# yml-bit/CTA-GAN

Measured on AMD Instinct MI355X. Metric: paired 512x512 slices/sec (G+D step); generator rel-L2 vs CPU reference, higher is better.
Workload: dtype bf16; 1 GPU; HdGan stage-2 full G+D train step (G, Reg, STN, D_m, losses, Adam x3), 16 paired 512x512 slices/GPU; per_gpu_batch=16, global_batch=16, size=512, parallelism=single, rccl_ranks=1, dp_backend=none

## Files before the change

### cta_gan_amd/csrc/conv_halo.h

```cpp
#pragma once
#include <stdlib.h>
#include <type_traits>
#include "common.h"
#include "conv_dispatch.h"

struct ConvArgs {
    const void* x;
    const void* w;
    void* y;
    const float* bias;
    int B, Hi, Wi, Cin, x_ld;
    int Ho, Wo, Cout, y_ld;
    int Hs, Ws, oy0, ox0, os, is;
    int frame;
    int pad_mode, act;
    int w_tap_stride;
    int ntaps;
    int taps[64];
    int kh, kw, dy0, dx0;
    float* stats;
    const void* res;
    const void* fold;
    int res_ld, fold_ld;
    const void* bz;
// ... 490 lines not shown
                                add_bf16x8(f, q); add_bf16x8(f, q + f_lo);
                            }
                        }
                    }
                    bf16x8 hi, lo;
#pragma unroll
                    for (int e = 0; e < 8; ++e) {
                        hi[e] = (bf16_t)f[e];
                        lo[e] = (bf16_t)(f[e] - (float)hi[e]);
                    }
                    bf16_t* yp = Y + (((size_t)n * a.Ho + (oy * a.os + oy0_)) * a.Wo + (ox * a.os + ox0_)) * a.y_ld + n0 + chl;
                    *reinterpret_cast<bf16x8*>(yp) = hi;
                    *reinterpret_cast<bf16x8*>(yp + y_lo) = lo;
                    if constexpr (FUSE) {
                        if (bst) {
                            const bf16_t* zp = Z + (((size_t)n * a.Hs + oy) * a.Ws + ox) * a.bz_ld + n0 + chl;
                            float zf[8];
#pragma unroll
                            for (int e = 0; e < 8; ++e) zf[e] = 0.f;
                            add_bf16x8(zf, zp);
                            add_bf16x8(zf, zp + z_lo);
#pragma unroll
                            for (int e = 0; e < 8; ++e) {
                                const float xh = (zf[e] - bmu[e]) * brs[e];
                                float gg = (float)hi[e] + (float)lo[e];
                                if (a.bact == ACT_RELU) gg = xh > 0.f ? gg : 0.f;
                                else if (a.bact == ACT_LRELU) gg = xh > 0.f ? gg : LRELU_SLOPE * gg;
                                bs1[e] += gg;
                                bs2[e] += gg * xh;
                            }
                        }
                    }
                }
            }
            if constexpr (FUSE) {
                if (bst) {
                    __syncthreads();
                    float* red = reinterpret_cast<float*>(smem);
#pragma unroll
                    for (int e = 0; e < 8; ++e) { red[tid * 16 + e] = bs1[e]; red[tid * 16 + 8 + e] = bs2[e]; }
                    __syncthreads();
                    const int ntile = gridDim.x / ntn;
                    for (int cl = tid; cl < CR; cl += NTH) {
                        const int ch = chan_of(cl, rd);
                        if (n0 + ch < a.Cout) {
                            float t1 = 0.f, t2 = 0.f;
                            for (int q = 0; q < NTH / CPR; ++q) {
                                const float* r = red + (q * CPR + (cl >> 3)) * 16 + (cl & 7);
                                t1 += r[0];
                                t2 += r[8];
                            }
                            float* dst = a.bstats + (((size_t)n * ntile + spc) * a.Cout + n0 + ch) * 2;
                            dst[0] = t1;
                            dst[1] = t2;
                        }
                    }
                }
            }
        }
    } else if constexpr (sizeof(OutT) == 2) {
        constexpr int RS = BN * 2 + 16;
        char* st = smem;
#pragma unroll
        for (int nt = 0; nt < TN; ++nt) {
            const int co = (wn * TN + nt) * 16 + co_l;
            float bv[4];
#pragma unroll
            for (int r = 0; r < 4; ++r)
                bv[r] = (a.bias != nullptr && n0 + co + r < a.Cout) ? a.bias[n0 + co + r] : 0.f;
#pragma unroll
            for (int mt = 0; mt < TM; ++mt) {
                const int prow = (wm * TM + mt) * HALO_W + (lane & 15);
                bf16x4 o;
#pragma unroll
                for (int r = 0; r < 4; ++r) {
                    if constexpr (NIE) o[r] = (bf16_t)act_apply((acc[mt][nt][r] - nmr[nt][r]) * nrr[nt][r], a.nie_act);
                    else o[r] = (bf16_t)act_apply(acc[mt][nt][r] + bv[r], a.act);
                }
                *reinterpret_cast<bf16x4*>(st + prow * RS + co * 2) = o;
            }
        }
        OutT* __restrict__ Y = (OutT*)a.y;
        const bf16_t* __restrict__ R = (const bf16_t*)a.res;
        const bf16_t* __restrict__ F = (const bf16_t*)a.fold;
        constexpr int CPR = BN / 8;
        constexpr int NIT = BM * CPR / NTH;
        u32x4 rv[FUSE ? NIT : 1], zv[FUSE ? NIT : 1];
        if constexpr (FUSE) {
#pragma unroll
            for (int it = 0; it < NIT; ++it) {
                const int cidx = tid + NTH * it;
                const int prow = cidx / CPR, ch = (cidx % CPR) * 8;
                const int oy = y0 + prow / HALO_W, ox = x0 + prow % HALO_W;
                const bool ok = R != nullptr && oy < a.Hs && ox < a.Ws && n0 + ch < a.Cout;
                rv[it] = *reinterpret_cast<const u32x4*>(
                    ok ? R + (((size_t)n * a.Hs + oy) * a.Ws + ox) * a.res_ld + n0 + ch : (const bf16_t*)g_zero_chunk);
                const bool okz = a.bstats != nullptr && oy < a.Hs && ox < a.Ws && n0 + ch < a.Cout;
                zv[it] = *reinterpret_cast<const u32x4*>(
                    okz ? (const bf16_t*)a.bz + (((size_t)n * a.Hs + oy) * a.Ws + ox) * a.bz_ld + n0 + ch : (const bf16_t*)g_zero_chunk);
            }
        }
        const bool bst = FUSE && a.bstats != nullptr;
        float bs1[8], bs2[8], bmu[8], brs[8];
#pragma unroll
        for (int e = 0; e < 8; ++e) { bs1[e] = 0.f; bs2[e] = 0.f; bmu[e] = 0.f; brs[e] = 0.f; }
        if constexpr (FUSE) {
            static_assert(NTH % CPR == 0, "a thread keeps its channel chunk over the store loop");
            const int chl = (tid % CPR) * 8;
            if (bst && n0 + chl < a.Cout) {
#pragma unroll
                for (int e = 0; e < 8; ++e) {
                    bmu[e] = a.bmean[(size_t)n * a.Cout + n0 + chl + e];
                    brs[e] = a.brstd[(size_t)n * a.Cout + n0 + chl + e];
                }
            }
        }
        __syncthreads();
#pragma unroll
        for (int it = 0; it < NIT; ++it) {
            const int cidx = tid + NTH * it;
            const int prow = cidx / CPR, ch = (cidx % CPR) * 8;
            const int oy = y0 + prow / HALO_W, ox = x0 + prow % HALO_W;
            if (oy < a.Hs && ox < a.Ws && n0 + ch < a.Cout) {
                OutT* yp = Y + (((size_t)n * a.Ho + (oy * a.os + oy0_)) * a.Wo + (ox * a.os + ox0_)) * a.y_ld + n0 + ch;
                u32x4 v = *reinterpret_cast<const u32x4*>(st + prow * RS + ch * 2);
                if constexpr (FUSE) {
                    float f[8], g[8];
                    unpack_bf16x8(v, f);
                    unpack_bf16x8(rv[it], g);
#pragma unroll
                    for (int e = 0; e < 8; ++e) f[e] += g[e];
                    if (F != nullptr) {
                        const int ey = oy == 1 ? 0 : (oy == a.Hs - 2 ? a.Hs + 1 : -1);
                        const int ex = ox == 1 ? 0 : (ox == a.Ws - 2 ? a.Ws + 1 : -1);
                        const OutT* Fn = F + (size_t)n * (a.Hs + 2) * (a.Ws + 2) * a.fold_ld + n0 + ch;
                        if (ey >= 0) add_bf16x8(f, Fn + ((size_t)ey * (a.Ws + 2) + ox + 1) * a.fold_ld);
                        if (ex >= 0) add_bf16x8(f, Fn + ((size_t)(oy + 1) * (a.Ws + 2) + ex) * a.fold_ld);
                        if (ey >= 0 && ex >= 0) add_bf16x8(f, Fn + ((size_t)ey * (a.Ws + 2) + ex) * a.fold_ld);
                    }
                    bf16x8 o;
#pragma unroll
                    for (int e = 0; e < 8; ++e) o[e] = (bf16_t)f[e];
                    v = __builtin_bit_cast(u32x4, o);
                    if (bst) {
                        float zf[8];
                        unpack_bf16x8(zv[it], zf);
#pragma unroll
                        for (int e = 0; e < 8; ++e) {
                            const float xh = (zf[e] - bmu[e]) * brs[e];
                            float gg = (float)o[e];
                            if (a.bact == ACT_RELU) gg = xh > 0.f ? gg : 0.f;
                            else if (a.bact == ACT_LRELU) gg = xh > 0.f ? gg : LRELU_SLOPE * gg;
                            bs1[e] += gg;
                            bs2[e] += gg * xh;
                        }
                    }
                }
                *reinterpret_cast<u32x4*>(yp) = v;
            }
        }
        if constexpr (FUSE) {
            if (bst) {
                __syncthreads();
                float* red = reinterpret_cast<float*>(smem);
#pragma unroll
                for (int e = 0; e < 8; ++e) { red[tid * 16 + e] = bs1[e]; red[tid * 16 + 8 + e] = bs2[e]; }
                __syncthreads();
                const int ntile = gridDim.x / ntn;
                for (int cl = tid; cl < BN; cl += NTH) {
                    if (n0 + cl < a.Cout) {
                        float t1 = 0.f, t2 = 0.f;
                        for (int q = 0; q < NTH / CPR; ++q) {
                            const float* r = red + (q * CPR + (cl >> 3)) * 16 + (cl & 7);
                            t1 += r[0];
                            t2 += r[8];
                        }
                        float* dst = a.bstats + (((size_t)n * ntile + spc) * a.Cout + n0 + cl) * 2;
                        dst[0] = t1;
                        dst[1] = t2;
                    }
                }
            }
        }
    } else {
        OutT* __restrict__ Y = (OutT*)a.y;
        const bool vec_ok = ((a.Cout & 3) == 0) && ((a.y_ld & 3) == 0);
#pragma unroll
        for (int mt = 0; mt < TM; ++mt) {
            const int oy = y0 + wm * TM + mt, ox = x0 + (lane & 15);
            if (oy >= a.Hs || ox >= a.Ws) continue;
            OutT* yp = Y + (((size_t)n * a.Ho + (oy * a.os + oy0_)) * a.Wo + (ox * a.os + ox0_)) * a.y_ld;
#pragma unroll
            for (int nt = 0; nt < TN; ++nt) {
                const int co = n0 + (wn * TN + nt) * 16 + co_l;
                if (co >= a.Cout) continue;
                float v[4];
#pragma unroll
                for (int r = 0; r < 4; ++r) {
                    const float b = (a.bias != nullptr && co + r < a.Cout) ? a.bias[co + r] : 0.f;
                    v[r] = act_apply(acc[mt][nt][r] + b, a.act);
                }
                if (FUSE && a.res != nullptr) {
                    const float* rp = (const float*)a.res + (((size_t)n * a.Hs + oy) * a.Ws + ox) * a.res_ld + co;
#pragma unroll
                    for (int r = 0; r < 4; ++r)
                        if (co + r < a.Cout) v[r] += rp[r];
                }
                if (FUSE && a.fold != nullptr) {
                    const int ey = oy == 1 ? 0 : (oy == a.Hs - 2 ? a.Hs + 1 : -1);
                    const int ex = ox == 1 ? 0 : (ox == a.Ws - 2 ? a.Ws + 1 : -1);
                    const float* Fn = (const float*)a.fold + (size_t)n * (a.Hs + 2) * (a.Ws + 2) * a.fold_ld + co;
#pragma unroll
                    for (int r = 0; r < 4; ++r) {
                        if (co + r >= a.Cout) continue;
                        if (ey >= 0) v[r] += Fn[((size_t)ey * (a.Ws + 2) + ox + 1) * a.fold_ld + r];
                        if (ex >= 0) v[r] += Fn[((size_t)(oy + 1) * (a.Ws + 2) + ex) * a.fold_ld + r];
                        if (ey >= 0 && ex >= 0) v[r] += Fn[((size_t)ey * (a.Ws + 2) + ex) * a.fold_ld + r];
                    }
                }
                if (vec_ok) {
                    *reinterpret_cast<f32x4*>(yp + co) = f32x4{v[0], v[1], v[2], v[3]};
                } else {
#pragma unroll
                    for (int r = 0; r < 4; ++r)
                        if (co + r < a.Cout) yp[co + r] = v[r];
                }
            }
        }
    }
}

template <typename T, typename OutT, int BN, int WM, int WN, int KCH, int ABUF, int TH = 16, bool FUSE = false, int KWC = 0, bool MC = false, bool PK = false,
          bool S2D = false, bool NIE = false>
static int launch_halo_cfg(const ConvArgs& a, hipStream_t st, int* tiles_out = nullptr) {
    if constexpr (!NIE && KWC == 3 && (TH == 16 || (TH == 8 && !PK)) && BN == 128 && WM == 4 && WN == 2 && KCH == 8 && !MC && !S2D &&
                  sizeof(T) == 2 && ((std::is_same<OutT, bf16_t>::value && !PK) || (std::is_same<OutT, bfpair_t>::value && PK))) {
        if (a.nie_sync != nullptr) {
            if ((FUSE && (a.fold != nullptr || a.bstats != nullptr)) || a.stats == nullptr || a.Cout % BN) return CTG_EINVAL;
            return launch_halo_cfg<T, OutT, BN, WM, WN, KCH, ABUF, TH, FUSE, KWC, false, PK, false, true>(a, st, tiles_out);
        }
    }
    if constexpr (!S2D && !FUSE && !MC && KWC == 0 && TH == 16 && sizeof(T) == 2 && KCH == 8 && BN >= 64 && !std::is_same<OutT, float>::value) {
        if (a.s2d) {
            if (a.res != nullptr || a.fold != nullptr) return -1;
            return launch_halo_cfg<T, OutT, BN, WM, WN, KCH, ABUF, TH, false, 0, false, PK, true>(a, st, tiles_out);
        }
    }
    if (a.s2d && !S2D) return -1;
    if constexpr (!FUSE && !MC && !S2D && !NIE) {
        if (a.res != nullptr || a.fold != nullptr) return launch_halo_cfg<T, OutT, BN, WM, WN, KCH, ABUF, TH, true, KWC, false, PK>(a, st, tiles_out);
    }
    if constexpr (!MC && !S2D && !FUSE && KWC == 0 && (TH == 16 || (TH == 8 && BN == 64)) && sizeof(T) == 2 &&
                  ((std::is_same<OutT, bf16_t>::value && !PK) || (std::is_same<OutT, bfpair_t>::value && PK))) {
        if (a.ncls == 4) return launch_halo_cfg<T, OutT, BN, WM, WN, KCH, ABUF, TH, false, 0, true, PK>(a, st, tiles_out);
    }
    if constexpr (KWC == 0 && !MC && !S2D && sizeof(T) == 2) {
        if (a.kw == 3 && a.kh <= 3 && a.ncls <= 1) return launch_halo_cfg<T, OutT, BN, WM, WN, KCH, ABUF, TH, FUSE, 3, false, PK>(a, st, tiles_out);
    }
    if (a.ncls > 1 && !MC && !S2D) return -1;
    if (a.nie_sync != nullptr && !NIE) return CTG_EINVAL;
    constexpr int NTH = WM * WN * 64;
    const int hpw = HALO_W + a.kw - 1, hph = TH + a.kh - 1;
    const int hpc = hph * hpw * KCH;
    const int hpc64 = (hpc + 63) & ~63;
    const int epc = VecOf<T>::N;
    const int nchunk = a.Cin / (KCH * epc);
    const int main_lds = (((nchunk > 1 && ABUF == 2) ? 2 : 1) * hpc64 + 2 * BN * KCH) * 16;
    const int epi_lds = std::is_same<OutT, bfpair_t>::value ? TH * HALO_W * ((BN / WN) * 4 + 16)
                        : sizeof(OutT) == 2 ? TH * HALO_W * (BN * 2 + 16) : 0;
    if (FUSE && a.bstats != nullptr && WM * WN * 64 * 64 > (main_lds > epi_lds ? main_lds : epi_lds)) return -1;
    const int smem = main_lds > epi_lds ? main_lds : epi_lds;
    if (smem > 160 * 1024 || hph * hpw >= 65536) return -1;
    static unsigned long long attr_mask = 0;
    {
        const int rc = ctg_lds_attr_once((const void*)conv_halo_kernel<T, OutT, BN, WM, WN, KCH, ABUF, TH, FUSE, KWC, MC, PK, S2D, NIE>,
                                         160 * 1024, &attr_mask);
        if (rc != CTG_OK) return rc;
    }
    const int tiles = ((a.Hs + TH - 1) / TH) * ((a.Ws + HALO_W - 1) / HALO_W) * (MC ? 4 : 1);
    if (tiles_out != nullptr) *tiles_out = tiles;
    const int ntn = (a.Cout + BN - 1) / BN;
    if constexpr (NIE) {
        static int occ_dev[64];
        int dev = 0;
        if (hipGetDevice(&dev) != hipSuccess) dev = 0;
        dev &= 63;
        if (occ_dev[dev] == 0) {
            int occ = 0;
            if (hipOccupancyMaxActiveBlocksPerMultiprocessor(
                    &occ, (const void*)conv_halo_kernel<T, OutT, BN, WM, WN, KCH, ABUF, TH, FUSE, KWC, MC, PK, S2D, NIE>, NTH, smem) != hipSuccess ||
                occ < 1)
                occ = 1;
            occ_dev[dev] = occ;
        }
        const int share = ctg_knobs().nie_share > 0 ? ctg_knobs().nie_share : 2;
        if ((long)tiles * ntn * share > (long)occ_dev[dev] * ctg_cu_count()) return 2;
    }
    dim3 grid(tiles * ntn, a.B);
    hipLaunchKernelGGL((conv_halo_kernel<T, OutT, BN, WM, WN, KCH, ABUF, TH, FUSE, KWC, MC, PK, S2D, NIE>), grid, dim3(NTH), smem, st, a);
    return ctg_launch_status();
}

static int launch_strip32(const ConvArgs& a, hipStream_t st, int* tiles_out, bool pair);

template <typename T, int KCH>
static int launch_halo_t(const ConvArgs& a, int out_f32, hipStream_t st, int* tiles_out) {
    if (a.is != 1 && !a.s2d) return -1;
    if (out_f32 >= 2) {
        if constexpr (sizeof(T) == 2 && KCH == 8) {
            if (out_f32 == 2) {
                if (a.Cout > 64) return launch_halo_cfg<T, bfpair_t, 128, 4, 2, 8, 1, 16, false, 0, false, true>(a, st, tiles_out);
                if (a.Cout > 32) {
                    if (a.ncls == 4 && !ctg_knobs().no_mc_th8) return launch_halo_cfg<T, bfpair_t, 64, 4, 1, 8, 1, 8, false, 0, false, true>(a, st, tiles_out);
                    if (!ctg_knobs().no_th8_64 && a.ncls <= 1 && a.Hs >= 16)
                        return launch_halo_cfg<T, bfpair_t, 64, 4, 1, 8, 1, 8, false, 0, false, true>(a, st, tiles_out);
                    return launch_halo_cfg<T, bfpair_t, 64, 4, 1, 8, 1, 16, false, 0, false, true>(a, st, tiles_out);
                }
                if (a.Cout > 16) {
                    const int rc = launch_strip32(a, st, tiles_out, true);
                    if (rc != -1) return rc;
                    return launch_halo_cfg<T, bfpair_t, 32, 4, 1, 8, 1, 16, false, 0, false, true>(a, st, tiles_out);
                }
                return -1;
            }
            if (a.Cout > 64) return launch_halo_cfg<T, float, 128, 4, 2, 8, 1, 16, false, 0, false, true>(a, st, tiles_out);
            if (a.Cout > 32) return launch_halo_cfg<T, float, 64, 4, 1, 8, 1, 16, false, 0, false, true>(a, st, tiles_out);
            if (a.Cout > 16) return launch_halo_cfg<T, float, 32, 4, 1, 8, 1, 16, false, 0, false, true>(a, st, tiles_out);
            return launch_halo_cfg<T, float, 16, 4, 1, 8, 1, 16, false, 0, false, true>(a, st, tiles_out);
        }
        return -1;
    }
    if (a.Cout > 64) {
        if (out_f32) {
            if constexpr (sizeof(T) == 2) return launch_halo_cfg<T, float, 128, 4, 2, KCH, 1>(a, st, tiles_out);
            return -1;
        }
        if constexpr (sizeof(T) == 2) {
            static_assert(HALO_W == 16, "halo_th8 counts 16-column tiles");
            if (halo_th8(a.Hs, a.Ws, a.Cout, a.B, a.ncls)) return launch_halo_cfg<T, T, 128, 4, 2, KCH, 1, 8>(a, st, tiles_out);
        }
        return launch_halo_cfg<T, T, 128, 4, 2, KCH, 1>(a, st, tiles_out);
    }
    if (a.Cout > 32) {
        if (out_f32) {
            if constexpr (sizeof(T) == 2) return launch_halo_cfg<T, float, 64, 4, 1, KCH, 1>(a, st, tiles_out);
            return -1;
        }
        if constexpr (sizeof(T) == 2 && KCH == 8) {
            if (!ctg_knobs().no_th8_64 && (a.ncls <= 1 || a.ncls == 4) && a.Hs >= 16) return launch_halo_cfg<T, T, 64, 4, 1, KCH, 1, 8>(a, st, tiles_out);
        }
        return launch_halo_cfg<T, T, 64, 4, 1, KCH, 1>(a, st, tiles_out);
    }
    if (a.Cout > 16) {
        if (out_f32) {
            if constexpr (sizeof(T) == 2) return launch_halo_cfg<T, float, 32, 4, 1, KCH, 1>(a, st, tiles_out);
            return -1;
        }
        if constexpr (sizeof(T) == 2 && KCH == 4) {
            const int rc = launch_strip32(a, st, tiles_out, false);
            if (rc != -1) return rc;
        }
        return launch_halo_cfg<T, T, 32, 4, 1, KCH, 1>(a, st, tiles_out);
    }
    if (out_f32 || sizeof(T) == 4) return launch_halo_cfg<T, float, 16, 4, 1, KCH, 1>(a, st, tiles_out);
    return -1;
}
```

### cta_gan_amd/csrc/conv_igemm.hip

```cpp
#include <stdlib.h>
#include "conv_halo.h"
#include "conv_strip.h"
#include "conv_stript.h"
#include "conv_pair_strips.h"
#include "conv_strips2.h"
#include "conv_strips2w.h"

__device__ __attribute__((aligned(16))) unsigned g_zero_chunk[4];

#ifndef CTG_BIG_TILE
#define CTG_BIG_TILE 1
#endif
static inline int gather_bm(bool bf16, bool k8, int omode, int Cout, long pixels) {
    return (bf16 && k8 && omode == 0 && Cout > 64 && pixels >= 4096 && CTG_BIG_TILE && !ctg_knobs().no_big_tile) ? 256 : 128;
}

#define FRAME_EDGE_PAD 128
__device__ __forceinline__ void grid_pixel(const ConvArgs& a, int m, int& j, int& i) {
    if (a.frame) {
        const int l1 = a.Hs - 2;
        const int p0 = (a.Ws + FRAME_EDGE_PAD - 1) & ~(FRAME_EDGE_PAD - 1), p1 = (l1 + FRAME_EDGE_PAD - 1) & ~(FRAME_EDGE_PAD - 1);
        if (m < p0) { j = 0; i = m < a.Ws ? m : a.Ws - 1; }
        else if (m < 2 * p0) { j = a.Hs - 1; i = m - p0 < a.Ws ? m - p0 : a.Ws - 1; }
        else {
            const int r = m - 2 * p0;
            if (r < p1) { j = (r < l1 ? r : l1 - 1) + 1; i = 0; }
            else { j = (r - p1 < l1 ? r - p1 : l1 - 1) + 1; i = a.Ws - 1; }
        }
    } else {
        j = m / a.Ws;
        i = m - j * a.Ws;
    }
}
__host__ __device__ __forceinline__ int grid_pixels(const ConvArgs& a) {
    if (a.frame)
        return 2 * ((a.Ws + FRAME_EDGE_PAD - 1) & ~(FRAME_EDGE_PAD - 1)) + 2 * ((a.Hs - 2 + FRAME_EDGE_PAD - 1) & ~(FRAME_EDGE_PAD - 1));
    return a.Hs * a.Ws;
}

template <typename T, typename OutT, int BM, int BN, int WM, int WN, int KCH, int NST, bool PK = false>
__global__ __launch_bounds__(WM * WN * 64) void conv_igemm_kernel(const ConvArgs a) {
    static_assert(!PK || (KCH == 8 && sizeof(T) == 2), "split-pair K steps (see ConvArgs::pair_lo)");
    constexpr int NTH = WM * WN * 64;
    constexpr int EPC = VecOf<T>::N;
    constexpr int BKE = KCH * EPC;
    constexpr int TM = BM / (WM * 16), TN = BN / (WN * 16);
    constexpr int A_CH = BM * KCH, B_CH = BN * KCH;
    constexpr int A_IT = A_CH / NTH, B_IT = (B_CH + NTH - 1) / NTH;
    static_assert(A_CH % NTH == 0 && (B_CH % NTH == 0 || B_CH < NTH) && B_CH % 64 == 0, "tile");
    static_assert(NST == 2 || (NST == 3 && B_CH % NTH == 0), "3-stage ring needs every wave to issue the same loads");
    extern __shared__ __attribute__((aligned(16))) char smem[];
    char* sA = smem;
    char* sB = smem + NST * A_CH * 16;

    const int tid = threadIdx.x, lane = tid & 63, wave = tid >> 6;
    const int wm = wave / WN, wn = wave % WN;
    const int n = blockIdx.y;
    const int ntn = (a.Cout + BN - 1) / BN;
    int id = blockIdx.x;
    id = xcd_contiguous(id, gridDim.x);
    const int m0 = (id / ntn) * BM, n0 = (id % ntn) * BN;
    const int Ms = grid_pixels(a);
    const T* __restrict__ X = (const T*)a.x;
    const T* __restrict__ W = (const T*)a.w;

    int aj[A_IT], ai[A_IT], akc[A_IT];
#pragma unroll
    for (int it = 0; it < A_IT; ++it) {
        const int s = tid + NTH * it;
        const int row = s / KCH;
        const int kcs = swz<KCH>(row, s % KCH);
        akc[it] = PK ? (kcs & 3) * EPC + (kcs >> 2) * a.pair_lo : kcs * EPC;
        int m = m0 + row;
        m = m < Ms ? m : Ms - 1;
        int j, i;
        grid_pixel(a, m, j, i);
        aj[it] = j * a.is;
        ai[it] = i * a.is;
    }
    int boff[B_IT];
    const bool b_active = (B_CH % NTH == 0) || (tid < B_CH);
#pragma unroll
    for (int it = 0; it < B_IT; ++it) {
        const int s = (tid + NTH * it) % B_CH;
        const int row = s / KCH;
        boff[it] = (n0 + row) * a.Cin + swz<KCH>(row, s % KCH) * EPC;
    }
    const int kPerTap = a.Cin / BKE;
    unsigned long long live = a.ntaps >= 64 ? ~0ull : ((1ull << a.ntaps) - 1ull);
    if (a.frame && a.pad_mode != PAD_REFLECT) {
        unsigned long long mine = 0ull;
        for (int t = 0; t < a.ntaps; ++t) {
            const int tw = a.taps[t];
            const int dy = (tw & 0xff) - 64, dx = ((tw >> 8) & 0xff) - 64;
            bool any = false;
#pragma unroll
            for (int it = 0; it < A_IT; ++it)
                any = any || (((unsigned)(aj[it] + dy) < (unsigned)a.Hi) && ((unsigned)(ai[it] + dx) < (unsigned)a.Wi));
            if (any) mine |= 1ull << t;
        }
        __shared__ unsigned long long live_s;
        if (tid == 0) live_s = 0ull;
        __syncthreads();
        if (mine) atomicOr(&live_s, mine);
        __syncthreads();
        live = live_s;
        if (live == 0ull) live = 1ull;
    }
    const int S = __popcll(live) * kPerTap;
    auto next_tap = [&]() __attribute__((always_inline)) {
        const int t = __ffsll((long long)live) - 1;
        live &= live - 1ull;
        return t;
    };

    long aoff[A_IT];
    int wbase = 0;
    auto set_tap = [&](int tap) __attribute__((always_inline)) {
        const int tw = a.taps[tap];
        const int dy = (tw & 0xff) - 64, dx = ((tw >> 8) & 0xff) - 64;
        wbase = (tw >> 16) * a.w_tap_stride;
#pragma unroll
        for (int it = 0; it < A_IT; ++it) {
            int iy = aj[it] + dy, ix = ai[it] + dx;
            bool ok = true;
            if (a.pad_mode == PAD_REFLECT) {
                iy = reflect_idx(iy, a.Hi);
                ix = reflect_idx(ix, a.Wi);
            } else {
                ok = ((unsigned)iy < (unsigned)a.Hi) && ((unsigned)ix < (unsigned)a.Wi);
            }
            aoff[it] = ok ? ((((long)n * a.Hi + iy) * a.Wi + ix) * a.x_ld + akc[it]) : -1L;
        }
    };
    auto issue = [&](int buf, int kc0) __attribute__((always_inline)) {
        const int xk = PK ? kc0 >> 1 : kc0;
#pragma unroll
        for (int it = 0; it < A_IT; ++it) {
            const T* src = aoff[it] >= 0 ? X + aoff[it] + xk : (const T*)g_zero_chunk;
            __builtin_amdgcn_global_load_lds((gptr_t)src, (lptr_t)(sA + (buf * A_CH + NTH * it + 64 * wave) * 16), 16, 0, 0);
        }
        if (b_active) {
#pragma unroll
            for (int it = 0; it < B_IT; ++it) {
                const T* src = W + wbase + boff[it] + kc0;
                __builtin_amdgcn_global_load_lds((gptr_t)src, (lptr_t)(sB + (buf * B_CH + NTH * it + 64 * wave) * 16), 16, 0, 0);
            }
        }
    };

    f32x4 acc[TM][TN];
#pragma unroll
    for (int i = 0; i < TM; ++i)
#pragma unroll
        for (int j = 0; j < TN; ++j) acc[i][j] = f32x4{0.f, 0.f, 0.f, 0.f};

    auto compute = [&](int buf) __attribute__((always_inline)) {
        const char* pa = sA + buf * A_CH * 16;
        const char* pb = sB + buf * B_CH * 16;
        if constexpr (PK) {
            u32x4 fa[TM], fb[TN], fl[TN];
            const int kc = lane >> 4;
#pragma unroll
            for (int mt = 0; mt < TM; ++mt) {
                const int row = (wm * TM + mt) * 16 + (lane & 15);
                fa[mt] = *reinterpret_cast<const u32x4*>(pa + (row * KCH + swz<KCH>(row, kc)) * 16);
            }
#pragma unroll
            for (int nt = 0; nt < TN; ++nt) {
                const int row = (wn * TN + nt) * 16 + (lane & 15);
                fb[nt] = *reinterpret_cast<const u32x4*>(pb + (row * KCH + swz<KCH>(row, kc)) * 16);
                fl[nt] = *reinterpret_cast<const u32x4*>(pb + (row * KCH + swz<KCH>(row, kc + 4)) * 16);
            }
#pragma unroll
            for (int mt = 0; mt < TM; ++mt)
#pragma unroll
                for (int nt = 0; nt < TN; ++nt) {
                    acc[mt][nt] = __builtin_amdgcn_mfma_f32_16x16x32_bf16(
                        __builtin_bit_cast(bf16x8, fb[nt]), __builtin_bit_cast(bf16x8, fa[mt]), acc[mt][nt], 0, 0, 0);
                    acc[mt][nt] = __builtin_amdgcn_mfma_f32_16x16x32_bf16(
                        __builtin_bit_cast(bf16x8, fl[nt]), __builtin_bit_cast(bf16x8, fa[mt]), acc[mt][nt], 0, 0, 0);
                }
#pragma unroll
            for (int mt = 0; mt < TM; ++mt) {
                const int row = (wm * TM + mt) * 16 + (lane & 15);
                fa[mt] = *reinterpret_cast<const u32x4*>(pa + (row * KCH + swz<KCH>(row, kc + 4)) * 16);
            }
#pragma unroll
            for (int mt = 0; mt < TM; ++mt)
#pragma unroll
                for (int nt = 0; nt < TN; ++nt)
                    acc[mt][nt] = __builtin_amdgcn_mfma_f32_16x16x32_bf16(
                        __builtin_bit_cast(bf16x8, fb[nt]), __builtin_bit_cast(bf16x8, fa[mt]), acc[mt][nt], 0, 0, 0);
        } else
#pragma unroll
        for (int ks = 0; ks < KCH / 4; ++ks) {
            u32x4 fa[TM], fb[TN];
            const int kc = ks * 4 + (lane >> 4);
#pragma unroll
            for (int mt = 0; mt < TM; ++mt) {
                const int row = (wm * TM + mt) * 16 + (lane & 15);
                fa[mt] = *reinterpret_cast<const u32x4*>(pa + (row * KCH + swz<KCH>(row, kc)) * 16);
            }
#pragma unroll
            for (int nt = 0; nt < TN; ++nt) {
                const int row = (wn * TN + nt) * 16 + (lane & 15);
                fb[nt] = *reinterpret_cast<const u32x4*>(pb + (row * KCH + swz<KCH>(row, kc)) * 16);
            }
#pragma unroll
            for (int mt = 0; mt < TM; ++mt)
#pragma unroll
                for (int nt = 0; nt < TN; ++nt) {
                    if constexpr (sizeof(T) == 2) {
                        acc[mt][nt] = __builtin_amdgcn_mfma_f32_16x16x32_bf16(
                            __builtin_bit_cast(bf16x8, fb[nt]), __builtin_bit_cast(bf16x8, fa[mt]), acc[mt][nt], 0, 0, 0);
                    } else {
                        const f32x4 va = __builtin_bit_cast(f32x4, fa[mt]);
                        const f32x4 vb = __builtin_bit_cast(f32x4, fb[nt]);
#pragma unroll
                        for (int q = 0; q < 4; ++q)
                            acc[mt][nt] = __builtin_amdgcn_mfma_f32_16x16x4f32(vb[q], va[q], acc[mt][nt], 0, 0, 0);
                    }
                }
        }
    };

    int kk = 0;
    auto advance = [&]() __attribute__((always_inline)) {
        if (++kk == kPerTap) {
            kk = 0;
            set_tap(next_tap());
        }
    };
    set_tap(next_tap());
    if constexpr (NST == 2) {
        issue(0, 0);
        __syncthreads();
        for (int s = 0; s < S; ++s) {
            const int cur = s & 1;
            if (s + 1 < S) {
                advance();
                issue(cur ^ 1, kk * BKE);
            }
            compute(cur);
            __syncthreads();
        }
    } else {
        constexpr int LOADS = A_IT + B_IT;
        issue(0, 0);
        if (S > 1) {
            advance();
            issue(1, kk * BKE);
        }
        int st = 0;
        for (int s = 0; s < S; ++s) {
            if (s + 1 < S) asm volatile("s_waitcnt vmcnt(%0)" ::"n"(LOADS) : "memory");
            else asm volatile("s_waitcnt vmcnt(0)" ::: "memory");
            __builtin_amdgcn_s_barrier();
            if (s + 2 < S) {
                advance();
                issue(st == 0 ? 2 : st - 1, kk * BKE);
            }
            compute(st);
            st = st == 2 ? 0 : st + 1;
        }
        __syncthreads();
    }

    const int co_l = (lane >> 4) * 4;
    if (a.stats != nullptr) {
        float* red = reinterpret_cast<float*>(smem);
#pragma unroll
        for (int nt = 0; nt < TN; ++nt) {
            float s1[4] = {0.f, 0.f, 0.f, 0.f}, s2[4] = {0.f, 0.f, 0.f, 0.f};
#pragma unroll
            for (int mt = 0; mt < TM; ++mt) {
                const bool valid = m0 + (wm * TM + mt) * 16 + (lane & 15) < Ms;
#pragma unroll
                for (int r = 0; r < 4; ++r) {
                    const float v = valid ? acc[mt][nt][r] : 0.f;
                    s1[r] += v;
                    s2[r] += v * v;
                }
            }
#pragma unroll
            for (int r = 0; r < 4; ++r) {
                s1[r] = row16_sum_to_lane15(s1[r]);
                s2[r] = row16_sum_to_lane15(s2[r]);
                if ((lane & 15) == 15) {
                    const int cl = (wn * TN + nt) * 16 + co_l + r;
                    red[(wm * BN + cl) * 2] = s1[r];
                    red[(wm * BN + cl) * 2 + 1] = s2[r];
                }
            }
        }
        __syncthreads();
        const int mtiles = gridDim.x / ntn;
        for (int cl = tid; cl < BN; cl += NTH) {
            if (n0 + cl < a.Cout) {
                float t1 = 0.f, t2 = 0.f;
#pragma unroll
                for (int w = 0; w < WM; ++w) { t1 += red[(w * BN + cl) * 2]; t2 += red[(w * BN + cl) * 2 + 1]; }
                float* dst = a.stats + (((size_t)n * mtiles + id / ntn) * a.Cout + n0 + cl) * 2;
                dst[0] = t1;
                dst[1] = t2;
// ... 457 lines not shown
```

### cta_gan_amd/csrc/ctg_knobs.h

```cpp
#pragma once
#include <stdlib.h>

namespace ctg_env {
static inline bool set(const char* name) { return getenv(name) != nullptr; }
static inline int num(const char* name, int dflt) { const char* v = getenv(name); return v ? atoi(v) : dflt; }
static inline long lnum(const char* name, long dflt) { const char* v = getenv(name); return v ? atol(v) : dflt; }
}

struct CtgKnobs {
    const bool no_halo = ctg_env::set("CTG_NO_HALO");
    const bool no_class_merge = ctg_env::set("CTG_NO_CLASS_MERGE");
    const bool no_s2d = ctg_env::set("CTG_NO_S2D");
    const bool no_nie = ctg_env::set("CTG_NO_NIE");
    const int nie_share = ctg_env::num("CTG_NIE_SHARE", 2);
    const bool no_th8 = ctg_env::set("CTG_NO_TH8");
    const long th8_wgs = ctg_env::lnum("CTG_TH8_WGS", 384);
    const bool no_th8_64 = ctg_env::set("CTG_NO_TH8_64");
    const bool no_mc_th8 = ctg_env::set("CTG_NO_MC_TH8");
    const bool no_big_tile = ctg_env::set("CTG_NO_BIG_TILE");
    const bool frame_bn128 = ctg_env::set("CTG_FRAME_BN128");
    const bool no_small_ring = ctg_env::set("CTG_NO_SMALL_RING");
    const bool no_strip = ctg_env::set("CTG_NO_STRIP");
    const int strip_band = ctg_env::num("CTG_STRIP_BAND", 0);
    const bool no_stript = ctg_env::set("CTG_NO_STRIPT");
    const int stript_band = ctg_env::num("CTG_STRIPT_BAND", 0);
    const int stript_xcd = ctg_env::num("CTG_STRIPT_XCD", 1);
    const bool no_striptp = ctg_env::set("CTG_NO_STRIPTP");
    const int striptp_band = ctg_env::num("CTG_STRIPTP_BAND", 0);
    const int striptp_wgs = ctg_env::num("CTG_STRIPTP_WGS", 1);
    const bool no_strips2 = ctg_env::set("CTG_NO_STRIPS2");
    const int strips2_band = ctg_env::num("CTG_STRIPS2_BAND", 0);
    const bool no_strips2p = ctg_env::set("CTG_NO_STRIPS2P");
    const int strips2p_band = ctg_env::num("CTG_STRIPS2P_BAND", 0);
    const bool no_strips2w = ctg_env::set("CTG_NO_STRIPS2W");
    const int strips2w_band = ctg_env::num("CTG_STRIPS2W_BAND", 0);
    const bool no_wg_1tap = ctg_env::set("CTG_NO_WG_1TAP");
    const bool no_wg_s2 = ctg_env::set("CTG_NO_WG_S2");
    const bool no_wg_s2m = ctg_env::set("CTG_NO_WG_S2M");
    const bool no_wg_phase_split = ctg_env::set("CTG_NO_WG_PHASE_SPLIT");
    const bool wg_noprefetch = ctg_env::set("CTG_WG_NOPREFETCH");
    const bool wg_noxcd = ctg_env::set("CTG_WG_NOXCD");
    const bool wg_no_reuse = ctg_env::set("CTG_WG_NO_REUSE");
    const int small_wgs = ctg_env::num("CTG_SMALL_WGS", 768);
    const bool no_smallb = ctg_env::set("CTG_NO_SMALLB");
};

static inline const CtgKnobs& ctg_knobs() {
    static const CtgKnobs k;
    return k;
}
```

Before: 333.9 slices/s.

## Add weight-stationary strip conv kernel for 3x3 bf16 convs with 32/64/96 channels

Adds a new 3x3 stride-1 convolution kernel that keeps all nine taps of weights in registers and streams 16-column strips of input rows through an LDS ring buffer via global_load_lds, with double-buffered LDS staging for coalesced output stores. It is dispatched ahead of the halo kernels for bf16 outputs with Cin/Cout pairs (96,32), (32,96), (64,64) on large images, optionally fusing bias+activation or BN statistics. The aim is to cut repeated weight loads and improve input reuse across rows. It adds heavy register pressure and hand-tuned waitcnt logic that could limit occupancy or be fragile.

```diff
diff --git a/cta_gan_amd/csrc/conv_halo.h b/cta_gan_amd/csrc/conv_halo.h
--- a/cta_gan_amd/csrc/conv_halo.h
+++ b/cta_gan_amd/csrc/conv_halo.h
@@ -816,6 +816,7 @@
 }
 
 static int launch_strip32(const ConvArgs& a, hipStream_t st, int* tiles_out, bool pair);
+static int launch_stripw(const ConvArgs& a, hipStream_t st, int* tiles_out);
 
 template <typename T, int KCH>
 static int launch_halo_t(const ConvArgs& a, int out_f32, hipStream_t st, int* tiles_out) {
@@ -844,6 +845,12 @@
         }
         return -1;
     }
+    if constexpr (sizeof(T) == 2) {
+        if (!out_f32) {
+            const int rc = launch_stripw(a, st, tiles_out);
+            if (rc != -1) return rc;
+        }
+    }
     if (a.Cout > 64) {
         if (out_f32) {
             if constexpr (sizeof(T) == 2) return launch_halo_cfg<T, float, 128, 4, 2, KCH, 1>(a, st, tiles_out);
diff --git a/cta_gan_amd/csrc/conv_igemm.hip b/cta_gan_amd/csrc/conv_igemm.hip
--- a/cta_gan_amd/csrc/conv_igemm.hip
+++ b/cta_gan_amd/csrc/conv_igemm.hip
@@ -1,6 +1,7 @@
 #include <stdlib.h>
 #include "conv_halo.h"
 #include "conv_strip.h"
+#include "conv_stripw.h"
 #include "conv_stript.h"
 #include "conv_pair_strips.h"
 #include "conv_strips2.h"
diff --git a/cta_gan_amd/csrc/conv_stripw.h b/cta_gan_amd/csrc/conv_stripw.h
--- /dev/null
+++ b/cta_gan_amd/csrc/conv_stripw.h
@@ -0,0 +1,317 @@
+#pragma once
+#include "conv_halo.h"
+#include "conv_strip.h"
+
+struct StripWArgs {
+    const bf16_t* x;
+    const bf16_t* w;
+    bf16_t* y;
+    const float* bias;
+    float* stats;
+    int B, H, W, x_ld, y_ld, w_tap_stride;
+    int pad_mode, act;
+    int band_rows, nbands, nstrips, xcd;
+    int widx[9];
+};
+
+template <int CIN, int COUT, int NG, int NTW, int RPW, int D>
+struct StripWCfg {
+    static constexpr int RG = 4 / NG;
+    static constexpr int SR = RG * RPW;
+    static constexpr int KS = CIN / 32;
+    static constexpr bool K8 = CIN % 64 == 0;
+    static constexpr int ROWB = 18 * CIN * 2;
+    static constexpr int CPR = ROWB / 16;
+    static constexpr int T = SR * CPR;
+    static constexpr int NI = (T + 255) / 256;
+    static constexpr int PS = T / (4 * NI);
+    static constexpr int NGR = D + 1;
+    static constexpr int RROWS = NGR * SR;
+    static constexpr int GROUPB = SR * ROWB;
+    static constexpr int STAGE = SR * 16 * COUT * 2;
+    static constexpr int NS = STAGE / 4096;
+    static constexpr int SMEM = NGR * GROUPB + 2 * STAGE;
+    static_assert(NG * NTW * 16 == COUT && NG * RG == 4 && CIN % 32 == 0, "wave layout");
+    static_assert(T % (4 * NI) == 0 && PS <= 64 && PS >= 1, "every wave issues NI DMA instructions with live lanes");
+    static_assert(STAGE % 4096 == 0, "whole-pixel stores: one 16-byte chunk per lane and pass");
+    static_assert(D >= 3, "a group is waited for two steps before the first step that reads all of it");
+    static_assert((D - 2) * (NI + NS) <= 63, "vmcnt is a 6-bit counter");
+};
+
+template <int CIN, int COUT, int NG, int NTW, int RPW, int D, bool FLIP, int MODE>
+__global__ __launch_bounds__(256, 2) void conv_stripw_kernel(const StripWArgs a) {
+    using C = StripWCfg<CIN, COUT, NG, NTW, RPW, D>;
+    constexpr bool EPI = MODE == 1, STATS = MODE == 2;
+    constexpr int SR = C::SR, KS = C::KS, NI = C::NI, NS = C::NS, PS = C::PS, ROWB = C::ROWB;
+    extern __shared__ __attribute__((aligned(16))) char smem[];
+    const int tid = threadIdx.x, lane = tid & 63, wave = __builtin_amdgcn_readfirstlane(tid >> 6);
+    const int p = lane & 15, kg = lane >> 4;
+    const int ng = wave % NG, rg = wave / NG;
+    const int item = a.xcd ? xcd_contiguous((int)blockIdx.x, (int)gridDim.x) : (int)blockIdx.x;
+    const int strip = item % a.nstrips;
+    const int t2 = item / a.nstrips;
+    const int band = t2 % a.nbands, n = t2 / a.nbands;
+    char* ring = smem;
+    char* stage = smem + C::NGR * C::GROUPB;
+    const int x0 = strip * 16, yb = band * a.band_rows;
+    const int nrows = min(a.band_rows, a.H - yb);
+    const int nsteps = (nrows + SR - 1) / SR;
+    const int H = a.H, W = a.W, x_ld = a.x_ld;
+    const char* __restrict__ Xn = reinterpret_cast<const char*>(a.x + (size_t)n * H * W * x_ld);
+
+    u32x4 wf[9][NTW][KS];
+#pragma unroll
+    for (int t = 0; t < 9; ++t)
+#pragma unroll
+        for (int nt = 0; nt < NTW; ++nt)
+#pragma unroll
+            for (int kk = 0; kk < KS; ++kk)
+                wf[t][nt][kk] = *reinterpret_cast<const u32x4*>(a.w + (size_t)a.widx[t] * a.w_tap_stride +
+                                                                ((ng * NTW + nt) * 16 + p) * CIN + kk * 32 + kg * 8);
+
+    int coloff[NI], rsel[NI];
+#pragma unroll
+    for (int k = 0; k < NI; ++k) {
+        const int q = (k * 4 + wave) * PS + (lane < PS ? lane : 0);
+        const int r = q / C::CPR, idx = q % C::CPR;
+        const int plane = idx / 72, rem = idx % 72;
+        const int px = rem >> 2, c = rem & 3;
+        int col = x0 - 1 + px;
+        if (a.pad_mode == PAD_REFLECT) col = reflect_idx(col, W);
+        const bool ok = (unsigned)col < (unsigned)W;
+        coloff[k] = ok ? (col * x_ld + plane * 32 + strip_swz(px, c) * 8) * 2 : -1;
+        rsel[k] = r;
+    }
+    const int rpitch = W * x_ld * 2;
+    auto issue_group = [&](int g) __attribute__((always_inline)) {
+        int rowoff[SR];
+#pragma unroll
+        for (int r = 0; r < SR; ++r) {
+            int row = yb - 1 + g * SR + r;
+            if (a.pad_mode == PAD_REFLECT) row = reflect_idx(row, H);
+            rowoff[r] = ((unsigned)row < (unsigned)H && g * SR + r < nrows + 2) ? row * rpitch : -1;
+        }
+        char* dst = ring + (g % C::NGR) * C::GROUPB + wave * (PS * 16);
+#pragma unroll
+        for (int k = 0; k < NI; ++k) {
+            int ro = rowoff[0];
+#pragma unroll
+            for (int r = 1; r < SR; ++r) ro = rsel[k] == r ? rowoff[r] : ro;
+            const char* src = (ro >= 0 && coloff[k] >= 0) ? Xn + ro + coloff[k] : reinterpret_cast<const char*>(g_zero_chunk);
+            if (PS == 64 || lane < PS) __builtin_amdgcn_global_load_lds((gptr_t)src, (lptr_t)(dst + k * (4 * PS * 16)), 16, 0, 0);
+        }
+    };
+
+    int loff[3];
+#pragma unroll
+    for (int k = 0; k < 3; ++k) {
+        const int px = p + k;
+        loff[k] = (px * 4 + strip_swz(px, kg)) * 16;
+    }
+    const bool col_ok = x0 + p < W;
+    const bool full_strip = x0 + 16 <= W;
+    float bv[EPI ? NTW : 1][4];
+    if constexpr (EPI) {
+#pragma unroll
+        for (int nt = 0; nt < NTW; ++nt)
+#pragma unroll
+            for (int r = 0; r < 4; ++r) bv[nt][r] = a.bias != nullptr ? a.bias[(ng * NTW + nt) * 16 + kg * 4 + r] : 0.f;
+    }
+    const float neg_slope = a.act == ACT_NONE ? 1.f : (a.act == ACT_RELU ? 0.f : LRELU_SLOPE);
+    float s1[NTW][4], s2[NTW][4];
+#pragma unroll
+    for (int nt = 0; nt < NTW; ++nt)
+#pragma unroll
+        for (int r = 0; r < 4; ++r) { s1[nt][r] = 0.f; s2[nt][r] = 0.f; }
+    static_assert(!STATS || C::RG == 1, "one slab per (band, strip): the waves of a workgroup hold different channels");
+
+    char* stage_w = stage + ((rg * RPW * 16 + p) * COUT + ng * NTW * 16 + kg * 4) * 2;
+    int st_row[NS];
+    bool st_colok[NS];
+    size_t st_off[NS];
+#pragma unroll
+    for (int i = 0; i < NS; ++i) {
+        const int q = tid + 256 * i;
+        const int pix = q / (COUT / 8), c = q % (COUT / 8);
+        st_row[i] = pix >> 4;
+        st_colok[i] = x0 + (pix & 15) < W;
+        st_off[i] = ((size_t)st_row[i] * W + (pix & 15)) * a.y_ld + c * 8;
+    }
+    bf16_t* __restrict__ yp = a.y + (((size_t)n * H + yb) * W + x0) * a.y_ld;
+    const size_t ystep = (size_t)SR * W * a.y_ld;
+
+#pragma unroll
+    for (int g = 0; g < D; ++g) issue_group(g);
+    asm volatile("s_waitcnt vmcnt(%0) lgkmcnt(0)" ::"n"((D - 2) * NI) : "memory");
+    __builtin_amdgcn_s_barrier();
+    asm volatile("" ::: "memory");
+
+    for (int j = 0; j < nsteps; ++j) {
+        issue_group(j + D);
+        const int par = j & 1;
+        {
+            const char* rrow[RPW + 2];
+            const int k0 = (j * SR + rg * RPW) % C::RROWS;
+#pragma unroll
+            for (int d = 0; d < RPW + 2; ++d) {
+                const int k = k0 + d >= C::RROWS ? k0 + d - C::RROWS : k0 + d;
+                rrow[d] = ring + k * ROWB;
+            }
+            f32x4 acc[RPW][NTW];
+#pragma unroll
+            for (int r = 0; r < RPW; ++r)
+#pragma unroll
+                for (int nt = 0; nt < NTW; ++nt) acc[r][nt] = f32x4{0.f, 0.f, 0.f, 0.f};
+            constexpr int KSUB = C::K8 ? 2 : 1;
+            u32x4 f[RPW + 2][3][KSUB];
+            auto load_row = [&](int d, int c) __attribute__((always_inline)) {
+#pragma unroll
+                for (int kx = 0; kx < 3; ++kx)
+#pragma unroll
+                    for (int ks = 0; ks < KSUB; ++ks)
+                        f[d][kx][ks] = *reinterpret_cast<const u32x4*>(rrow[d] + (c * KSUB + ks) * 1152 + loff[kx]);
+            };
+            constexpr int NSL = KS / KSUB;
+#pragma unroll
+            for (int r = 0; r < RPW; ++r) load_row((FLIP ? 2 : 0) + r, 0);
+#pragma unroll
+            for (int c = 0; c < NSL; ++c) {
+#pragma unroll
+                for (int s = 0; s < 3; ++s) {
+                    const int ky = FLIP ? 2 - s : s;
+                    if (s < 2) {
+                        load_row(FLIP ? ky - 1 : ky + RPW, c);
+                    } else if (c + 1 < NSL) {
+                        static_assert(RPW <= 2, "the first rows of the next slice go where no MFMA of the last kernel row reads");
+#pragma unroll
+                        for (int r = 0; r < RPW; ++r) load_row((FLIP ? 2 : 0) + r, c + 1);
+                    }
+                    __builtin_amdgcn_sched_barrier(0);
+#pragma unroll
+                    for (int kxs = 0; kxs < 3; ++kxs) {
+                        const int kx = FLIP ? 2 - kxs : kxs;
+                        const int t = s * 3 + kxs;
+#pragma unroll
+                        for (int ks = 0; ks < KSUB; ++ks)
+#pragma unroll
+                            for (int r = 0; r < RPW; ++r)
+#pragma unroll
+                                for (int nt = 0; nt < NTW; ++nt)
+                                    acc[r][nt] = __builtin_amdgcn_mfma_f32_16x16x32_bf16(__builtin_bit_cast(bf16x8, wf[t][nt][c * KSUB + ks]),
+                                                                                         __builtin_bit_cast(bf16x8, f[r + ky][kx][ks]),
+                                                                                         acc[r][nt], 0, 0, 0);
+                    }
+                }
+            }
+#pragma unroll
+            for (int r = 0; r < RPW; ++r)
+#pragma unroll
+                for (int nt = 0; nt < NTW; ++nt) asm volatile("" : "+v"(acc[r][nt]));
+            asm volatile("s_nop 7\n\ts_nop 7" ::: "memory");
+#pragma unroll
+            for (int r = 0; r < RPW; ++r)
+#pragma unroll
+                for (int nt = 0; nt < NTW; ++nt) asm volatile("" : "+v"(acc[r][nt]));
+#pragma unroll
+            for (int r = 0; r < RPW; ++r) {
+#pragma unroll
+                for (int nt = 0; nt < NTW; ++nt) {
+                    bf16x4 o;
+#pragma unroll
+                    for (int e = 0; e < 4; ++e) {
+                        float v = acc[r][nt][e];
+                        if constexpr (EPI) {
+                            v += bv[nt][e];
+                            v = v > 0.f ? v : v * neg_slope;
+                        }
+                        o[e] = (bf16_t)v;
+                    }
+                    *reinterpret_cast<bf16x4*>(stage_w + par * C::STAGE + (r * 16 * COUT + nt * 16) * 2) = o;
+                }
+                if constexpr (STATS) {
+                    const bool ok = col_ok && j * SR + rg * RPW + r < nrows;
+#pragma unroll
+                    for (int nt = 0; nt < NTW; ++nt)
+#pragma unroll
+                        for (int e = 0; e < 4; ++e) {
+                            const float v = ok ? acc[r][nt][e] : 0.f;
+                            s1[nt][e] += v;
+                            s2[nt][e] += v * v;
+                        }
+                }
+            }
+        }
+        if (!full_strip || j + 1 >= nsteps) asm volatile("s_waitcnt vmcnt(0) lgkmcnt(0)" ::: "memory");
+        else if (j < D - 2) asm volatile("s_waitcnt vmcnt(%0) lgkmcnt(0)" ::"n"((D - 2) * NI) : "memory");
+        else asm volatile("s_waitcnt vmcnt(%0) lgkmcnt(0)" ::"n"((D - 2) * (NI + NS)) : "memory");
+        __builtin_amdgcn_s_barrier();
+        asm volatile("" ::: "memory");
+#pragma unroll
+        for (int i = 0; i < NS; ++i) {
+            const u32x4 o = *reinterpret_cast<const u32x4*>(stage + par * C::STAGE + (tid + 256 * i) * 16);
+            if (st_colok[i] && j * SR + st_row[i] < nrows) *reinterpret_cast<u32x4*>(yp + st_off[i]) = o;
+        }
+        yp += ystep;
+    }
+    asm volatile("s_waitcnt vmcnt(0)" ::: "memory");
+    if constexpr (STATS) {
+        const int slab = band * a.nstrips + strip, slabs = a.nbands * a.nstrips;
+        float* dst = a.stats + (((size_t)n * slabs + slab) * COUT) * 2;
+#pragma unroll
+        for (int nt = 0; nt < NTW; ++nt)
+#pragma unroll
+            for (int e = 0; e < 4; ++e) {
+                const float t1 = row16_sum_to_lane15(s1[nt][e]), t2v = row16_sum_to_lane15(s2[nt][e]);
+                if (p == 15) {
+                    const int ch = (ng * NTW + nt) * 16 + kg * 4 + e;
+                    dst[ch * 2] = t1;
+                    dst[ch * 2 + 1] = t2v;
+                }
+            }
+    }
+}
+
+template <int CIN, int COUT, int NG, int NTW, int RPW, int D>
+static int launch_stripw_cfg(const ConvArgs& a, hipStream_t st, int* tiles_out, int band_env) {
+    using C = StripWCfg<CIN, COUT, NG, NTW, RPW, D>;
+    const bool fwd = taps_3x3(a.taps, false);
+    if (!fwd && !taps_3x3(a.taps, true)) return -1;
+    const bool epi = a.bias != nullptr || a.act != ACT_NONE;
+    if (a.stats != nullptr && (epi || C::RG != 1)) return -1;
+    StripWArgs s;
+    s.x = (const bf16_t*)a.x; s.w = (const bf16_t*)a.w; s.y = (bf16_t*)a.y; s.bias = a.bias; s.stats = a.stats;
+    s.B = a.B; s.H = a.Hs; s.W = a.Ws; s.x_ld = a.x_ld; s.y_ld = a.y_ld; s.w_tap_stride = a.w_tap_stride;
+    s.pad_mode = a.pad_mode; s.act = a.act;
+    s.nstrips = (a.Ws + 15) / 16;
+    s.xcd = 1;
+    const BandPlan bp = band_plan(a.Hs, 16, 2L * ctg_cu_count(), (long)a.B * s.nstrips, band_env);
+    s.band_rows = bp.band_rows;
+    s.nbands = bp.nbands;
+    for (int t = 0; t < 9; ++t) s.widx[t] = a.taps[t] >> 16;
+    if (tiles_out != nullptr) *tiles_out = s.nbands * s.nstrips;
+    const dim3 grid((unsigned)((long)a.B * s.nbands * s.nstrips));
+    const int mode = epi ? 1 : (a.stats != nullptr ? 2 : 0);
+#define STRIPW_LAUNCH(FLIP, MODE) launch_lds<conv_stripw_kernel<CIN, COUT, NG, NTW, RPW, D, FLIP, MODE>>(grid, dim3(256), C::SMEM, st, s)
+    if constexpr (C::RG == 1) {
+        if (mode == 2) return fwd ? STRIPW_LAUNCH(false, 2) : STRIPW_LAUNCH(true, 2);
+    }
+    if (mode == 1) return fwd ? STRIPW_LAUNCH(false, 1) : STRIPW_LAUNCH(true, 1);
+    return fwd ? STRIPW_LAUNCH(false, 0) : STRIPW_LAUNCH(true, 0);
+#undef STRIPW_LAUNCH
+}
+
+static int launch_stripw(const ConvArgs& a, hipStream_t st, int* tiles_out) {
+    if (a.kh != 3 || a.kw != 3 || a.ntaps != 9 || a.is != 1 || a.os != 1 || a.ncls > 1 || a.s2d || a.frame || a.oy0 != 0 || a.ox0 != 0 ||
+        a.Ho != a.Hs || a.Wo != a.Ws || a.Hi != a.Hs || a.Wi != a.Ws || a.res != nullptr || a.fold != nullptr || a.bstats != nullptr ||
+        a.nie_sync != nullptr || a.pair_lo != 0 || a.dy0 != -1 || a.dx0 != -1 || a.act > ACT_LRELU)
+        return -1;
+    if ((long)a.B * a.Hs * a.Ws < (1L << 20) || a.Hs < 32 || a.Ws < 32 || (a.y_ld & 7) || (a.x_ld & 7)) return -1;
+    if ((long)a.Hs * a.Ws * a.x_ld * 2 >= (1L << 31)) return -1;
+    if (a.Cin == 96 && a.Cout == 32 && !ctg_knobs().no_stripw_96_32)
+        return launch_stripw_cfg<96, 32, 2, 1, 2, 4>(a, st, tiles_out, ctg_knobs().stripw_96_32_band);
+    if (a.Cin == 32 && a.Cout == 96 && !ctg_knobs().no_stripw_32_96)
+        return launch_stripw_cfg<32, 96, 2, 3, 2, 8>(a, st, tiles_out, ctg_knobs().stripw_32_96_band);
+    if (a.Cin == 64 && a.Cout == 64 && !ctg_knobs().no_stripw_64_64)
+        return launch_stripw_cfg<64, 64, 4, 1, 2, 8>(a, st, tiles_out, ctg_knobs().stripw_64_64_band);
+    return -1;
+}
diff --git a/cta_gan_amd/csrc/ctg_knobs.h b/cta_gan_amd/csrc/ctg_knobs.h
--- a/cta_gan_amd/csrc/ctg_knobs.h
+++ b/cta_gan_amd/csrc/ctg_knobs.h
@@ -34,6 +34,12 @@
     const int strips2p_band = ctg_env::num("CTG_STRIPS2P_BAND", 0);
     const bool no_strips2w = ctg_env::set("CTG_NO_STRIPS2W");
     const int strips2w_band = ctg_env::num("CTG_STRIPS2W_BAND", 0);
+    const bool no_stripw_96_32 = ctg_env::set("CTG_NO_STRIPW_96_32");
+    const int stripw_96_32_band = ctg_env::num("CTG_STRIPW_96_32_BAND", 0);
+    const bool no_stripw_32_96 = ctg_env::set("CTG_NO_STRIPW_32_96");
+    const int stripw_32_96_band = ctg_env::num("CTG_STRIPW_32_96_BAND", 0);
+    const bool no_stripw_64_64 = ctg_env::set("CTG_NO_STRIPW_64_64");
+    const int stripw_64_64_band = ctg_env::num("CTG_STRIPW_64_64_BAND", 0);
     const bool no_wg_1tap = ctg_env::set("CTG_NO_WG_1TAP");
     const bool no_wg_s2 = ctg_env::set("CTG_NO_WG_S2");
     const bool no_wg_s2m = ctg_env::set("CTG_NO_WG_S2M");
```

Result: no change. 336.5 slices/s, median of 6 (+0.8%).
